# lezhnev74/inverted_index_2

Hardware: NVIDIA B200
Metric: merged postings/s (higher is better)
Workload: dtype u32

## Files before the change

inverted_index_2_b200/csrc/k12_fused.cu:

```cuda
#include "keys.cuh"
#include "union_dev.cuh"

namespace ii2 {

constexpr int F_THREADS = 512;
constexpr int F_MIN_CTAS = 2;
constexpr int F_WARPS = F_THREADS / 32;
constexpr uint32_t F_CAP_I = 1024;
constexpr int F_PER = (F_CAP_I + F_THREADS - 1) / F_THREADS;
constexpr uint32_t F_HT = F_CAP_I > 512 ? 2048 : 1024;
constexpr uint32_t F_A_CH = F_CAP_I * 5 / 4;
constexpr uint32_t F_C_CH = F_CAP_I;
constexpr uint32_t F_B_CH = F_CAP_I * 9 / 8;
constexpr uint32_t F_ARENA_W = (F_A_CH + F_C_CH) * 4;
constexpr uint32_t F_GCAP = F_CAP_I * 4;
constexpr uint32_t F_SMALL_D = 64;
constexpr uint32_t F_EMPTY = 0xFFFFFFFFu;
static_assert(F_CAP_I <= 1024 && F_CAP_I % 64 == 0 && F_THREADS >= 128 && F_THREADS % 32 == 0 &&
              F_HT >= 2 * F_CAP_I, "tile shape");
static_assert(F_B_CH * 16 < 65536, "term positions inside the staged bytes are 16-bit");
static_assert(F_ARENA_W < (1u << 14) && F_GCAP < (1u << 13), "packed output prefixes");

__host__ __device__ inline size_t k12f_smem_bytes(int k) {
  return (size_t)(F_A_CH + F_C_CH + F_B_CH) * 16 + 64
// ... 352 lines not shown
    }
  } else {
    bitonic_sort_any(reps, D, tid, (uint32_t)F_THREADS, less, [] { __syncthreads(); });
    __syncthreads();
    uint32_t run_p = 0, run_e = 0;
    for (uint32_t base = 0; base < D; base += F_THREADS) {
      const uint32_t r = base + tid;
      uint32_t me = 0, li = 0, ei = 0;
      if (r < D) {
        me = reps[r];
        const uint32_t len = cg[me] & 0xFFFFFu;
        if (len > REG_CAP) s_bad = 1;
        li = (len + 3u) & ~3u;
        ei = enc_slot_words(len);
      }
      uint32_t tp, te;
      const uint32_t xp = block_exclusive_scan(li, s_ws32, tp);
      const uint32_t xe = block_exclusive_scan(ei, s_ws32, te);
      if (r < D) {
        order[r] = (uint16_t)me;
        pbase[me] = run_p + xp;
        ebase[me] = run_e + xe;
        if (li >= 128)
          wide_list[atomicAdd(&s_nw, 1u)] = (uint16_t)r;
        else
          narrow_list[atomicAdd(&s_nn, 1u)] = (uint16_t)r;
      }
      run_p += tp;
      run_e += te;
    }
    if (tid == 0) {
      s_tot[0] = run_p;
      s_tot[1] = run_e;
    }
  }
  __syncthreads();
  if (s_bad || s_tot[0] > F_GCAP || (a.want_enc && s_tot[1] > F_ARENA_W)) {
    defer();
    return;
  }

#pragma unroll
  for (int j = 0; j < F_PER; j++) {
    const uint32_t i = tid + j * F_THREADS;
    if (i < W) {
      const uint32_t g = og[j] >> 20;
      const uint32_t* src = reinterpret_cast<const uint32_t*>(smem + ps[j]);
      uint32_t* dst = gather + pbase[g] + (og[j] & 0xFFFFFu);
      const uint32_t n = pl[j];
      uint32_t t = 0;
#pragma unroll 1
      for (; t + 4 <= n; t += 4) {
        const uint32_t x0 = src[t], x1 = src[t + 1], x2 = src[t + 2], x3 = src[t + 3];
        dst[t] = x0;
        dst[t + 1] = x1;
        dst[t + 2] = x2;
        dst[t + 3] = x3;
      }
      if (t < n) {
        const uint32_t x0 = src[t];
        const uint32_t x1 = t + 1 < n ? src[t + 1] : 0u;
        const uint32_t x2 = t + 2 < n ? src[t + 2] : 0u;
        dst[t] = x0;
        if (t + 1 < n) dst[t + 1] = x1;
        if (t + 2 < n) dst[t + 2] = x2;
      }
    }
  }
  __syncthreads();

  uint32_t* const arena = reinterpret_cast<uint32_t*>(smem + OFF_A);
  {
    const unsigned half = lane >> 4, hl = lane & 15u;
    const uint32_t nw = s_nw, nn = s_nn;
    const uint32_t items = nw + ((nn + 1) >> 1);
#pragma unroll 1
    for (uint32_t it = warp; it < items; it += F_WARPS) {
      if (it < nw) {
        const uint32_t r = wide_list[it];
        const uint32_t me = order[r];
        const uint32_t c = cg[me];
        uint32_t* const wslot = gather + pbase[me];
        uint32_t* const weslot = arena + ebase[me];
        const uint32_t outn = union_blocked<32>(wslot, wslot, c & 0xFFFFFu, (c >> 20) > 1, a.rem);
        uint32_t enc = 0;
        if (a.want_enc && outn) enc = encode_shared_warp(wslot, outn, weslot);
        if (lane == 0) rres[r] = outn | (enc << 16);
      } else {
        const uint32_t q = 2 * (it - nw) + half;
        const bool has = q < nn;
        const uint32_t r = has ? narrow_list[q] : 0u;
        const uint32_t me = has ? order[r] : 0u;
        const uint32_t c = has ? cg[me] : 0u;
        uint32_t* const slot = gather + (has ? pbase[me] : 0u);
        uint32_t* const eslot = arena + (has ? ebase[me] : 0u);
        const uint32_t outn = union_blocked<16>(slot, slot, c & 0xFFFFFu, (c >> 20) > 1, a.rem);
        uint32_t enc = 0;
        if (a.want_enc) enc = encode_small_blocked<16>(slot, outn, eslot);
        if (has && hl == 0) rres[r] = outn | (enc << 16);
      }
      __syncwarp();
    }
  }
  __syncthreads();

  const bool keep_empty = a.keep_empty != 0;
  auto packed = [&](uint32_t r) -> uint64_t {
    const uint32_t res = rres[r];
    const uint32_t cnt = res & 0xFFFFu, enc = res >> 16;
    if (!(cnt || keep_empty)) return 0ull;
    return 1ull | ((uint64_t)cnt << 11) | ((uint64_t)enc << 24) | ((uint64_t)tlen[order[r]] << 38);
  };
  if (D <= 64) {
    if (warp == 0) {
      const uint64_t v0 = lane < D ? packed(lane) : 0ull;
      const uint64_t v1 = lane + 32 < D ? packed(lane + 32) : 0ull;
      const uint64_t i0 = warp_inclusive_scan(v0);
      const uint64_t t0 = __shfl_sync(0xffffffffu, i0, 31);
      const uint64_t i1 = warp_inclusive_scan(v1) + t0;
      if (lane < D) pfx[lane] = i0 - v0;
      if (lane + 32 < D) pfx[lane + 32] = i1 - v1;
      if (lane == 31) s_total = i1;
    }
  } else {
    uint64_t run = 0;
    for (uint32_t base = 0; base < D; base += F_THREADS) {
      const uint32_t r = base + tid;
      const uint64_t v = r < D ? packed(r) : 0ull;
      uint64_t tot;
      const uint64_t ex = block_exclusive_scan(v, s_ws64, tot);
      if (r < D) pfx[r] = run + ex;
      run += tot;
    }
    if (tid == 0) s_total = run;
  }
  __syncthreads();
  {
    const uint64_t P0 = a.bk_P[b], E0 = a.bk_E[b], T0 = a.bk_TB[b];
    uint8_t* const o_tb = a.st_tb + T0;
    uint32_t* const o_enc = a.st_enc + E0;
    uint32_t* const o_post = a.st_post + P0;
#pragma unroll 1
    for (uint32_t r = warp; r < D; r += F_WARPS) {
      const uint32_t res = rres[r];
      const uint32_t cnt = res & 0xFFFFu, enc = res >> 16;
      if (!(cnt || keep_empty)) continue;
      const uint32_t me = order[r];
      const uint64_t x = pfx[r];
      const uint32_t t = (uint32_t)x & 0x7FFu, po = (uint32_t)(x >> 11) & 0x1FFFu,
                     eo = (uint32_t)(x >> 24) & 0x3FFFu, to = (uint32_t)(x >> 38);
      const uint32_t n = tlen[me];
      if (lane == 0) {
        a.st_toff[rec_base + t] = to;
        if (a.want_enc) a.st_eoff[rec_base + t] = eo;
        if (a.want_dec) a.st_poff[rec_base + t] = po;
      }
      const uint8_t* tsrc = smem + OFF_B + tsm[me];
      for (uint32_t i = lane; i < n; i += 32) o_tb[to + i] = tsrc[i];
      if (a.want_enc) {
        const uint32_t* esrc = arena + ebase[me];
        for (uint32_t i = lane; i < enc; i += 32) o_enc[eo + i] = esrc[i];
      }
      if (a.want_dec) {
        const uint32_t* dsrc = gather + pbase[me];
        for (uint32_t i = lane; i < cnt; i += 32) o_post[po + i] = dsrc[i];
      }
    }
  }
  if (tid == 0) {
    const uint64_t x = s_total;
    a.bk_D[b] = D;
    a.bk_mode[b] = K12F_DENSE;
    a.bk_raw[0ull * a.nb1 + b] = x & 0x7FFu;
    a.bk_raw[1ull * a.nb1 + b] = x >> 38;
    a.bk_raw[2ull * a.nb1 + b] = (x >> 11) & 0x1FFFu;
    a.bk_raw[3ull * a.nb1 + b] = (x >> 24) & 0x3FFFu;
  }
}

bool k12f_supported(int k) {
  return k >= 1 && k <= (int)F_MAXK && 4 * k <= (int)F_CAP_I && k <= F_THREADS;
// ... 17 lines not shown
```

inverted_index_2_b200/csrc/k12_union.cu:

```cuda
#include <algorithm>
#include <cstdlib>
#include <vector>

#include "intcomp.cuh"
#include "keys.cuh"
#include "union.cuh"
#include "union_dev.cuh"

namespace ii2 {

constexpr int K1B_THREADS = 256;
constexpr int K1B_WARPS = K1B_THREADS / 32;
constexpr uint32_t CAP_I = 1024;
constexpr uint32_t K1B_HT = CAP_I > 512 ? 2048 : 1024;
static_assert(CAP_I % K1B_THREADS == 0 && CAP_I <= 1024 && CAP_I % 4 == 0,
              "tile = a whole number of instances per thread, 10-bit tile indexes");
constexpr uint32_t K1B_STAGE_CAP = CAP_I * 6;
constexpr uint32_t K1B_SMALL_D = 64;
constexpr uint32_t K1B_EMPTY = 0xFFFFFFFFu;
constexpr uint32_t K12_PENDING = 0xFFFFFFFFu;
constexpr uint32_t K1B_HEAVY = 0xFFFFFFFFu;

struct K1bArgs {
  const SegDesc* segs;
// ... 393 lines not shown
      if (tid == 0) {
        s_tot[0] = run_p;
        s_tot[1] = run_e;
      }
    }
    __syncthreads();

    const uint32_t tile_p = s_tot[0];
    const bool staged = tile_p <= K1B_STAGE_CAP;
    uint32_t* const stage = reinterpret_cast<uint32_t*>(key_hi);
    auto copy_source = [](const uint32_t* __restrict__ src, uint32_t* __restrict__ dst, uint32_t n) {
      uint32_t t = 0;
#pragma unroll 1
      for (; t + 4 <= n; t += 4) {
        const uint32_t x0 = __ldg(src + t), x1 = __ldg(src + t + 1), x2 = __ldg(src + t + 2),
                       x3 = __ldg(src + t + 3);
        dst[t] = x0;
        dst[t + 1] = x1;
        dst[t + 2] = x2;
        dst[t + 3] = x3;
      }
      if (t < n) {
        const uint32_t x0 = __ldg(src + t);
        const uint32_t x1 = t + 1 < n ? __ldg(src + t + 1) : 0u;
        const uint32_t x2 = t + 2 < n ? __ldg(src + t + 2) : 0u;
        dst[t] = x0;
        if (t + 1 < n) dst[t + 1] = x1;
        if (t + 2 < n) dst[t + 2] = x2;
      }
    };
#pragma unroll
    for (int j = 0; j < PER; j++) {
      const uint32_t i = tid + j * K1B_THREADS;
      if (i < size) {
        const uint32_t g = og[j] >> 20;
        const uint32_t pb = pbase[g];
        if (pb != K1B_HEAVY) {
          const uint32_t* src = reinterpret_cast<const uint32_t*>(pp[j]);
          const uint32_t at = pb + (og[j] & 0xFFFFFu);
          if (staged)
            copy_source(src, stage + (at - pcount), pl[j]);
          else
            copy_source(src, gath + at, pl[j]);
        } else {
          const uint32_t at = sbase[g] + ((atomicSub(&cg[g], 1u << 20) >> 20) - 1u);
          a.src_ptr[at] = pp[j];
          a.src_len[at] = pl[j];
        }
      }
    }
    if (staged) {
      __syncthreads();
      uint32_t* const out = gath + pcount;
      const uint32_t head = min(tile_p, (uint32_t)((16u - ((uintptr_t)out & 15u)) & 15u) >> 2);
      if (tid < head) out[tid] = stage[tid];
      const uint32_t nvec = (tile_p - head) >> 2;
      for (uint32_t v = tid; v < nvec; v += K1B_THREADS) {
        const uint32_t e = head + 4 * v;
        *reinterpret_cast<uint4*>(out + e) =
            make_uint4(stage[e], stage[e + 1], stage[e + 2], stage[e + 3]);
      }
      const uint32_t tail0 = head + 4 * nvec;
      if (tail0 + tid < tile_p) out[tail0 + tid] = stage[tail0 + tid];
    }
    dcount += D;
    icount += size;
    pcount += s_tot[0];
    ecount += s_tot[1];
    W -= size;
    if (W == 0) break;
    __syncthreads();
    for (int s = tid; s < k; s += K1B_THREADS) cur[s] = mmp[s];
    __syncthreads();
  }
  if (tid == 0) a.bk_D[b] = dcount;
}


constexpr int K2B_THREADS = 128;
constexpr int K2B_WARPS = K2B_THREADS / 32;
constexpr uint32_t K2B_HALF = 128;
constexpr uint32_t K2B_ENC_WORDS = 3 + 2 * 129 + 1 + (5 * 127 + 3) / 4 + 1;
constexpr uint32_t K2B_EBUF = (K2B_ENC_WORDS + 7) & ~7u;
static_assert(K2B_EBUF / 2 >= 1 + (5 * 127 + 3) / 4, "var-byte stream of 127 values fits a half");

struct K2bArgs {
  const uint64_t* bk_pos;
  const uint64_t* bk_P;
  const uint64_t* bk_E;
  const uint32_t* bk_D;
  const GroupIn* gin;
  RemovedSet rem;
  int want_enc, want_dec, keep_empty;
  GroupRec* recs;
  uint32_t* gath;
  uint32_t* tmp_enc;
  uint64_t* bk_raw;
  uint32_t nb1;
  uint32_t* n_large;
  uint32_t* large_rec;
  uint32_t* large_bucket;
  uint32_t bucket0;
  const uint32_t* list;
};

constexpr int K2B_MIN_CTAS = 8;
template <bool LIST>
__global__ void __launch_bounds__(K2B_THREADS, K2B_MIN_CTAS) k2b_union_kernel(const K2bArgs a) {
  pdl_enter();
  __shared__ __align__(16) uint32_t s_buf[K2B_WARPS][REG_CAP];
  __shared__ __align__(16) uint32_t s_enc[K2B_WARPS][K2B_EBUF];
  const unsigned lane = lane_id(), warp = warp_id();
  const unsigned half = lane >> 4, hl = lane & 15u;
  const uint32_t b = LIST ? a.list[blockIdx.x] : a.bucket0 + blockIdx.x;
  const uint32_t D = a.bk_D[b];
  if (D == 0) return;
  const uint64_t rec_base = a.bk_pos[b];
  uint32_t* const gath = a.gath + a.bk_P[b];
  uint32_t* const enc_base = a.tmp_enc + a.bk_E[b];
  uint32_t acc_t = 0, acc_tb = 0, acc_e = 0;
  uint64_t acc_p = 0;
  const GroupIn g_none = {0u, 0u, 0u, 0u, 0u, 0u, 0u, 0u};
  GroupIn g_next = g_none;
  if (2 * warp + half < D) g_next = a.gin[rec_base + 2 * warp + half];
#pragma unroll 1
  for (uint32_t p0 = 2 * warp; p0 < D; p0 += 2 * K2B_WARPS) {
    const uint32_t r = p0 + half;
    const bool has = r < D;
    const GroupIn g = g_next;
    {
      const uint32_t rn = r + 2 * K2B_WARPS;
      g_next = g_none;
      if (rn < D) g_next = a.gin[rec_base + rn];
    }

    const bool heavy = has && g.L > REG_CAP;
    const bool wide = has && !heavy && g.L >= K2B_HALF;
    if (heavy && hl == 0) {
      const uint32_t slot = atomicAdd(a.n_large, 1u);
      a.large_rec[slot] = (uint32_t)(rec_base + r);
      a.large_bucket[slot] = b;
      GroupRec rec;
      rec.inst = g.inst;
      rec.tlen = g.tlen;
      rec.dec = 0;
      rec.eoff = 0;
      rec.enc = 0;
      rec.cnt = K12_PENDING;
      a.recs[rec_base + r] = rec;
    }
    {
      const bool mine = has && !heavy && !wide;
      const uint32_t L = mine ? g.L : 0u;
      uint32_t* const slot = gath + g.pst;
      uint32_t* const buf = s_buf[warp] + half * K2B_HALF;
      uint32_t* const ebuf = s_enc[warp] + half * (K2B_EBUF / 2);
      const uint32_t outn = union_blocked<16>(slot, buf, L, g.c > 1, a.rem);
      if (a.want_dec)
        for (uint32_t e = hl; e < outn; e += 16) slot[e] = buf[e];
      uint32_t enc = 0;
      uint32_t* const enc_dst = enc_base + g.eslot;
      if (a.want_enc) {
        enc = encode_small_blocked<16>(buf, outn, ebuf);
        for (uint32_t e = hl; e < enc; e += 16) enc_dst[e] = ebuf[e];
      }
      if (mine && hl == 0) {
        GroupRec rec;
        rec.inst = g.inst;
        rec.tlen = g.tlen;
        rec.dec = reinterpret_cast<uint64_t>(slot);
        rec.eoff = a.want_enc ? reinterpret_cast<uint64_t>(enc_dst) : 0ull;
        rec.cnt = outn;
        rec.enc = enc;
        a.recs[rec_base + r] = rec;
        if (outn || a.keep_empty) {
          acc_t += 1;
          acc_tb += g.tlen;
          acc_p += outn;
          acc_e += enc;
        }
      }
      __syncwarp();
    }
    unsigned wmask = __ballot_sync(0xffffffffu, wide && hl == 0);
    while (wmask) {
      const int src = __ffs(wmask) - 1;
      wmask &= wmask - 1;
      GroupIn w;
      w.inst = __shfl_sync(0xffffffffu, g.inst, src);
      w.tlen = __shfl_sync(0xffffffffu, g.tlen, src);
      w.c = __shfl_sync(0xffffffffu, g.c, src);
      w.L = __shfl_sync(0xffffffffu, g.L, src);
      w.pst = __shfl_sync(0xffffffffu, g.pst, src);
      w.eslot = __shfl_sync(0xffffffffu, g.eslot, src);
      const uint32_t rw = p0 + (src >> 4);
      uint32_t* const slot = gath + w.pst;
      uint32_t* const buf = s_buf[warp];
      uint32_t* const ebuf = s_enc[warp];
      const uint32_t outn = union_blocked<32>(slot, buf, w.L, w.c > 1, a.rem);
      if (a.want_dec)
        for (uint32_t e = lane; e < outn; e += 32) slot[e] = buf[e];
      uint32_t enc = 0;
      uint32_t* const enc_dst = enc_base + w.eslot;
      if (a.want_enc && outn) {
        enc = encode_shared_warp(buf, outn, ebuf);
        for (uint32_t e = lane; e < enc; e += 32) enc_dst[e] = ebuf[e];
      }
      if (lane == 0) {
        GroupRec rec;
        rec.inst = w.inst;
        rec.tlen = w.tlen;
        rec.dec = reinterpret_cast<uint64_t>(slot);
        rec.eoff = a.want_enc ? reinterpret_cast<uint64_t>(enc_dst) : 0ull;
        rec.cnt = outn;
        rec.enc = enc;
        a.recs[rec_base + rw] = rec;
        if (outn || a.keep_empty) {
          acc_t += 1;
          acc_tb += w.tlen;
          acc_p += outn;
          acc_e += enc;
        }
      }
      __syncwarp();
    }
  }
  if (hl == 0 && acc_t) {
    unsigned long long* bo = reinterpret_cast<unsigned long long*>(a.bk_raw);
    atomicAdd(&bo[0ull * a.nb1 + b], (unsigned long long)acc_t);
    atomicAdd(&bo[1ull * a.nb1 + b], (unsigned long long)acc_tb);
    atomicAdd(&bo[2ull * a.nb1 + b], (unsigned long long)acc_p);
    atomicAdd(&bo[3ull * a.nb1 + b], (unsigned long long)acc_e);
  }
}

constexpr uint32_t MW_CAP = 1024;
constexpr int MW_V = 32;
constexpr int MW_WARPS = 4;
constexpr int MW_MIN_CTAS = 5;
constexpr uint32_t MW_BUF = MW_CAP + MW_CAP / 32 + 8;
constexpr uint32_t MW_EBUF = 3 + 8 * 129 + 1 + 1 + 6;
static_assert(MW_EBUF >= kMaxSegs + 1, "source prefix fits the stream buffer");

struct MwArgs {
  const uint32_t* n_in_list;
  const uint32_t* in_rec;
  const uint32_t* in_bucket;
  const GroupIn* gin;
  const uint64_t* src_ptr;
  const uint32_t* src_len;
  GroupRec* recs;
  RemovedSet rem;
  int want_enc, keep_empty;
  uint64_t* bk_raw;
  uint32_t nb1;
  uint32_t* cursor;
  uint32_t* n_out_list;
  uint32_t* out_rec;
  uint32_t* out_bucket;
  uint32_t* out_post;
  uint32_t* out_enc;
  unsigned long long* out_cursor;
};

__global__ void __launch_bounds__(MW_WARPS * 32, MW_MIN_CTAS) k2_mwarp_kernel(const MwArgs a) {
  pdl_enter();
  __shared__ __align__(16) uint32_t s_buf[MW_WARPS][MW_BUF];
  __shared__ __align__(16) uint32_t s_enc[MW_WARPS][MW_EBUF];
  const unsigned lane = lane_id(), warp = warp_id();
  uint32_t* const buf = s_buf[warp];
  uint32_t* const ebuf = s_enc[warp];
  uint32_t* const moff = ebuf;
  for (;;) {
    uint32_t item = 0;
    if (lane == 0) item = atomicAdd(a.cursor, 1u);
    item = __shfl_sync(0xffffffffu, item, 0);
    if (item >= *a.n_in_list) return;
    const uint32_t rec = a.in_rec[item], bucket = a.in_bucket[item];
    const GroupIn g = a.gin[rec];
    const uint32_t c = g.c, beg = g.src;
    uint32_t run = 0;
    for (uint32_t base = 0; base < c; base += 32) {
      const uint32_t i = base + lane;
      uint32_t li = i < c ? a.src_len[beg + i] : 0u;
      li = li > MW_CAP + 1 ? MW_CAP + 1 : li;
      const uint32_t inc = warp_inclusive_scan(li);
      if (i < c) moff[i] = min(run + inc - li, MW_CAP + 1);
      run = min(run + __shfl_sync(0xffffffffu, inc, 31), MW_CAP + 1);
    }
    if (run > MW_CAP) {
      if (lane == 0) {
        const uint32_t at = atomicAdd(a.n_out_list, 1u);
        a.out_rec[at] = rec;
        a.out_bucket[at] = bucket;
      }
      continue;
// ... 774 lines not shown
  II2_TRY(u.recs.alloc_scratch(N, s));
  II2_TRY(u.bk_D.alloc_scratch(B, s));
  II2_TRY(u.bk_raw.alloc_scratch(4 * (size_t)(B + 1), s));
  II2_TRY(u.bk_out.alloc_scratch(4 * (size_t)(B + 1), s));
  II2_TRY(u.totals.alloc_scratch(8, s));
  const uint64_t enc_cap = n_in + n_in / 4 + 6ull * N + 64;
  if (want_enc) II2_TRY(u.tmp_enc.alloc_scratch(enc_cap, s, 16));
  II2_TRY(u.tmp_post.alloc_scratch(n_in, s, 16));
  const uint32_t large_cap = (uint32_t)std::min<uint64_t>(N, n_in / REG_CAP + 1);
  DevBuf<uint32_t> large_u32;
  II2_TRY(large_u32.alloc_scratch(8 * (size_t)large_cap, s));
  DevBuf<unsigned long long> med_cursor;
  II2_TRY(med_cursor.alloc_scratch(8, s));
  II2_CUDA_TRY(cudaMemsetAsync(med_cursor.p, 0, 64, s));
  II2_TRY(u.med_post.alloc_scratch(n_in, s, 16));
  if (want_enc) II2_TRY(u.med_enc.alloc_scratch(n_in + n_in / 4 + 16ull * large_cap + 64, s, 16));
  II2_CUDA_TRY(cudaMemsetAsync(u.totals.p, 0, 64, s));
  II2_CUDA_TRY(cudaMemsetAsync(u.bk_raw.p, 0, 4 * (size_t)(B + 1) * 8, s));
  II2_TRY(u.bk_mode.alloc_scratch(B, s));
  if (u.fused) {
    II2_TRY(u.st_tb.alloc_scratch(tb_in, s, 64));
    II2_TRY(u.st_off.alloc_scratch(3 * (size_t)N, s));
    II2_TRY(u.def_list.alloc_scratch(B, s));
  } else {
    II2_CUDA_TRY(cudaMemsetAsync(u.bk_mode.p, 0, (size_t)B * 4, s));
  }

  K1bArgs a1;
  a1.segs = plan.segs;
  a1.k = k;
  a1.part = plan.part.p;
  a1.btb = plan.btb.p;
  a1.bpo = plan.bpo.p;
  a1.bk_pos = plan.bk_pos();
  a1.bk_cpl = plan.bk_cpl.p;
  a1.bk_P = plan.bk_P();
  a1.gin = gin.p;
  a1.gath = u.tmp_post.p;
  a1.src_ptr = src_ptr.p;
  a1.src_len = src_len.p;
  a1.bk_D = u.bk_D.p;
  K2bArgs a2;
  a2.bk_pos = plan.bk_pos();
  a2.bk_P = plan.bk_P();
  a2.bk_E = plan.bk_E();
  a2.bk_D = u.bk_D.p;
  a2.gin = gin.p;
  a2.rem = rem;
  a2.want_enc = want_enc ? 1 : 0;
  a2.want_dec = want_dec ? 1 : 0;
  a2.keep_empty = keep_empty ? 1 : 0;
  a2.recs = u.recs.p;
  a2.gath = u.tmp_post.p;
  a2.tmp_enc = u.tmp_enc.p;
  a2.bk_raw = u.bk_raw.p;
  a2.nb1 = B + 1;
  a2.n_large = reinterpret_cast<uint32_t*>(u.totals.p + 6);
  a2.large_rec = large_u32.p;
  a2.large_bucket = large_u32.p + large_cap;
  const size_t smem = k1b_smem_bytes(k);
  static size_t attr = 0;
  if (smem > attr) {
    const size_t want = std::max(k1b_smem_bytes(kMaxSegs), smem);
    II2_CUDA_TRY(cudaFuncSetAttribute(k1b_group_kernel<false>, cudaFuncAttributeMaxDynamicSharedMemorySize,
                                      (int)want));
    II2_CUDA_TRY(cudaFuncSetAttribute(k1b_group_kernel<true>, cudaFuncAttributeMaxDynamicSharedMemorySize,
                                      (int)want));
    attr = want;
  }
  auto general = [&](uint32_t grid, const uint32_t* list) -> int {
    a1.bucket0 = a2.bucket0 = 0;
    a1.list = a2.list = list;
    {
      ProfScope scope("k1b_group", s);
      if (list) {
        II2_LAUNCH_CHAIN(k1b_group_kernel<true>, grid, K1B_THREADS, smem, s, a1);
      } else {
        II2_LAUNCH_CHAIN(k1b_group_kernel<false>, grid, K1B_THREADS, smem, s, a1);
      }
    }
    {
      ProfScope scope("k2b_union", s);
      if (list) {
        II2_LAUNCH_CHAIN(k2b_union_kernel<true>, grid, K2B_THREADS, 0, s, a2);
      } else {
        II2_LAUNCH_CHAIN(k2b_union_kernel<false>, grid, K2B_THREADS, 0, s, a2);
      }
    }
    {
      ProfScope scope("k2_medium", s);
      uint32_t* const mid_rec = large_u32.p + 4 * (size_t)large_cap;
      uint32_t* const mid_bucket = large_u32.p + 5 * (size_t)large_cap;
      uint32_t* const n_mid = reinterpret_cast<uint32_t*>(med_cursor.p + 3);
      MwArgs w2;
      w2.n_in_list = a2.n_large;
      w2.in_rec = a2.large_rec;
      w2.in_bucket = a2.large_bucket;
      w2.gin = gin.p;
      w2.src_ptr = src_ptr.p;
      w2.src_len = src_len.p;
      w2.recs = u.recs.p;
      w2.rem = rem;
      w2.want_enc = want_enc ? 1 : 0;
      w2.keep_empty = keep_empty ? 1 : 0;
      w2.bk_raw = u.bk_raw.p;
      w2.nb1 = B + 1;
      w2.cursor = reinterpret_cast<uint32_t*>(med_cursor.p + 2) + 1;
      w2.n_out_list = n_mid;
      w2.out_rec = mid_rec;
      w2.out_bucket = mid_bucket;
      w2.out_post = u.med_post.p;
      w2.out_enc = u.med_enc.p;
      w2.out_cursor = med_cursor.p;
      II2_LAUNCH_CHAIN(k2_mwarp_kernel, kNumSMs * MW_MIN_CTAS, MW_WARPS * 32, 0, s, w2);
      uint32_t* const mid2_rec = large_u32.p + 6 * (size_t)large_cap;
      uint32_t* const mid2_bucket = large_u32.p + 7 * (size_t)large_cap;
      uint32_t* const n_mid2 = reinterpret_cast<uint32_t*>(med_cursor.p + 3) + 1;
      MedArgs m;
      m.n_large = n_mid;
      m.large_rec = mid_rec;
      m.large_bucket = mid_bucket;
      m.gin = gin.p;
      m.src_ptr = src_ptr.p;
      m.src_len = src_len.p;
      m.recs = u.recs.p;
      m.rem = rem;
      m.want_enc = want_enc ? 1 : 0;
      m.keep_empty = keep_empty ? 1 : 0;
      m.bk_raw = u.bk_raw.p;
      m.nb1 = B + 1;
      m.cursor = reinterpret_cast<uint32_t*>(med_cursor.p + 4);
      m.n_huge = n_mid2;
      m.huge_rec = mid2_rec;
      m.huge_bucket = mid2_bucket;
      m.out_post = u.med_post.p;
      m.out_enc = u.med_enc.p;
      m.out_cursor = med_cursor.p;
      II2_LAUNCH_CHAIN(k2_medium_kernel<4>, kNumSMs * 8, 4 * 32, 0, s, m);
      m.n_large = n_mid2;
      m.large_rec = mid2_rec;
      m.large_bucket = mid2_bucket;
      m.cursor = reinterpret_cast<uint32_t*>(med_cursor.p + 2);
      m.n_huge = a2.n_large + 1;
      m.huge_rec = large_u32.p + 2 * (size_t)large_cap;
      m.huge_bucket = large_u32.p + 3 * (size_t)large_cap;
      II2_LAUNCH_CHAIN(k2_medium_kernel<8>, kNumSMs * 5, 8 * 32, 0, s, m);
    }
    return II2_OK;
  };
  uint64_t* h_tot = pinned_scratch();
  if (!h_tot) return II2_ERR_NOMEM;
  auto totals = [&](bool emit_early = false) -> int {
    ProfScope scope("k12_scan_sync", s);
    II2_TRY(exclusive_scan_multi_sum_to_host(u.bk_raw.p, u.bk_out.p, B + 1, 4, u.totals.p, u.bk_D.p, B,
                                             4, h_tot, 8, s));
    if (emit_early) II2_TRY(k6_emit_early(plan, u, n_in, tb_in, *u.early_out, s));
    II2_CUDA_TRY(cudaStreamSynchronize(s));
    return II2_OK;
  };
  if (u.fused) {
    K12fArgs f;
    f.segs = plan.segs;
    f.k = k;
    f.part = plan.part.p;
    f.btb = plan.btb.p;
    f.bpo = plan.bpo.p;
    f.bk_pos = plan.bk_pos();
    f.bk_cpl = plan.bk_cpl.p;
    f.bk_P = plan.bk_P();
// ... 59 lines not shown
```

inverted_index_2_b200/csrc/union_dev.cuh:

```cuda
#pragma once
#include "intcomp.cuh"
#include "union.cuh"

namespace ii2 {

constexpr uint32_t REG_CAP = 256;

__host__ __device__ __forceinline__ uint32_t enc_slot_words(uint32_t n) { return n + (n >> 2) + 6; }

__device__ __forceinline__ void cex(uint32_t& x, uint32_t& y) {
  const uint32_t lo = min(x, y), hi = max(x, y);
  x = lo;
  y = hi;
}

__device__ __forceinline__ void sort8_local(uint32_t (&v)[8]) {
  cex(v[0], v[1]); cex(v[2], v[3]); cex(v[4], v[5]); cex(v[6], v[7]);
  cex(v[0], v[2]); cex(v[1], v[3]); cex(v[4], v[6]); cex(v[5], v[7]);
  cex(v[1], v[2]); cex(v[5], v[6]); cex(v[0], v[4]); cex(v[3], v[7]);
  cex(v[1], v[5]); cex(v[2], v[6]);
  cex(v[1], v[4]); cex(v[3], v[6]);
  cex(v[2], v[4]); cex(v[3], v[5]);
  cex(v[3], v[4]);
}
// ... 32 lines not shown
  if (nmax > 8) merge_level<16>(v, hl);
  if (nmax > 16) merge_level<32>(v, hl);
  if (nmax > 32) merge_level<64>(v, hl);
  if (nmax > 64) merge_level<128>(v, hl);
  if (W == 32 && nmax > 128) merge_level<256>(v, hl);
}

template <int V>
__device__ __forceinline__ void sort_local_v(uint32_t (&v)[V]) {
#pragma unroll
  for (int k = 2; k <= V; k <<= 1) {
#pragma unroll
    for (int j = k >> 1; j > 0; j >>= 1) {
#pragma unroll
      for (int i = 0; i < V; i++) {
        const int l = i ^ j;
        if (l > i) {
          const uint32_t lo = min(v[i], v[l]), hi = max(v[i], v[l]);
          const bool asc = (i & k) == 0;
          v[i] = asc ? lo : hi;
          v[l] = asc ? hi : lo;
        }
      }
    }
  }
}

template <int V>
__device__ __forceinline__ void clean_local_v(uint32_t (&v)[V]) {
#pragma unroll
  for (int d = V / 2; d > 0; d >>= 1) {
#pragma unroll
    for (int i = 0; i < V; i++)
      if ((i & d) == 0) cex(v[i], v[i + d]);
  }
}

template <int V>
__device__ __forceinline__ void sort_warp_v(uint32_t (&v)[V], unsigned lane, uint32_t n) {
  sort_local_v<V>(v);
#pragma unroll 1
  for (uint32_t K = 2 * V; K <= 32 * V && n > K / 2; K <<= 1) {
    {
      const unsigned dist = K / V - 1;
      const bool lower = (lane & (K / (2 * V))) == 0;
#pragma unroll
      for (int r = 0; r < V / 2; r++) {
        const uint32_t a = v[r], b = v[V - 1 - r];
        const uint32_t oa = __shfl_xor_sync(0xffffffffu, b, dist);
        const uint32_t ob = __shfl_xor_sync(0xffffffffu, a, dist);
        v[r] = ((a < oa) == lower) ? a : oa;
        v[V - 1 - r] = ((b < ob) == lower) ? b : ob;
      }
    }
#pragma unroll 1
    for (uint32_t j = K / 4; j >= V; j >>= 1) {
      const unsigned dist = j / V;
      const bool lower = (lane & dist) == 0;
#pragma unroll
      for (int r = 0; r < V; r++) {
        const uint32_t o = __shfl_xor_sync(0xffffffffu, v[r], dist);
        v[r] = ((v[r] < o) == lower) ? v[r] : o;
      }
    }
    clean_local_v<V>(v);
  }
}

template <int V>
__device__ __forceinline__ void clean_warp_v(uint32_t (&v)[V], unsigned lane) {
#pragma unroll 1
  for (unsigned dist = 16; dist >= 1; dist >>= 1) {
    const bool lower = (lane & dist) == 0;
#pragma unroll
    for (int r = 0; r < V; r++) {
      const uint32_t o = __shfl_xor_sync(0xffffffffu, v[r], dist);
      v[r] = ((v[r] < o) == lower) ? v[r] : o;
    }
  }
  clean_local_v<V>(v);
}

template <int W>
__device__ __forceinline__ uint32_t union_blocked(const uint32_t* slot, uint32_t* buf, uint32_t L,
                                                  bool multi, const RemovedSet& rem) {
  const unsigned lane = lane_id(), hl = lane & (W - 1);
  uint32_t v[8];
#pragma unroll
  for (int r = 0; r < 8; r++) {
    const uint32_t e = hl * 8 + r;
    v[r] = e < L ? slot[e] : 0xFFFFFFFFu;
  }
  const bool any_multi = __any_sync(0xffffffffu, multi && L > 1);
  if (any_multi) {
    const uint32_t nmax = __reduce_max_sync(0xffffffffu, multi ? L : 0u);
    sort_blocked<W>(v, hl, nmax);
    if (!multi) {
#pragma unroll
      for (int r = 0; r < 8; r++) {
        const uint32_t e = hl * 8 + r;
        v[r] = e < L ? slot[e] : 0xFFFFFFFFu;
      }
    }
  }
  uint32_t keep = 0;
  if (rem.bitmap) {
    const uint32_t nbits = (uint32_t)rem.bitmap_bits;
    uint32_t word[8];
#pragma unroll
    for (int r = 0; r < 8; r++) {
      const bool probe = hl * 8 + r < L && v[r] < nbits;
      word[r] = probe ? __ldg(rem.bitmap + (v[r] >> 5)) : 0u;
    }
#pragma unroll
    for (int r = 0; r < 8; r++)
      keep |= (hl * 8 + r < L && !((word[r] >> (v[r] & 31u)) & 1u)) ? 1u << r : 0u;
  } else {
#pragma unroll
    for (int r = 0; r < 8; r++)
      if (hl * 8 + r < L && !is_removed(rem, v[r])) keep |= 1u << r;
  }
  const uint32_t up = __shfl_up_sync(0xffffffffu, v[7], 1, W);
  if (multi) {
    if (hl > 0 && up == v[0]) keep &= ~1u;
#pragma unroll
    for (int r = 1; r < 8; r++)
      if (v[r] == v[r - 1]) keep &= ~(1u << r);
  }
  const uint32_t cnt = __popc(keep);
  uint32_t inc = cnt;
#pragma unroll
  for (int d = 1; d < W; d <<= 1) {
    const uint32_t o = __shfl_up_sync(0xffffffffu, inc, d, W);
    if (hl >= (unsigned)d) inc += o;
  }
  const uint32_t outn = __shfl_sync(0xffffffffu, inc, W - 1, W);
  uint32_t* dst = buf + (inc - cnt);
#pragma unroll
  for (int r = 0; r < 8; r++) {
    const bool k = (keep >> r) & 1u;
    if (k) *dst = v[r];
    dst += k ? 1 : 0;
  }
  __syncwarp();
  return outn;
}

template <int W>
__device__ __forceinline__ uint32_t encode_small_blocked(const uint32_t* v, uint32_t n,
                                                         uint32_t* out) {
  const unsigned hl = lane_id() & (W - 1);
  const uint32_t e0 = hl * 8;
  const uint4 a = *reinterpret_cast<const uint4*>(v + e0);
  const uint4 b = *reinterpret_cast<const uint4*>(v + e0 + 4);
  const uint32_t x[8] = {a.x, a.y, a.z, a.w, b.x, b.y, b.z, b.w};
  uint32_t prev = e0 ? v[e0 - 1] : 0u;
  uint32_t z[8], lens = 0, bytes = 0;
#pragma unroll
  for (int r = 0; r < 8; r++) {
    z[r] = intcomp::zigzag(x[r], prev);
    prev = x[r];
    const uint32_t bl = 32u - __clz(z[r] | 1u);
    const uint32_t len = e0 + r < n ? ((bl + 6u) * 37u) >> 8 : 0u;
    lens |= len << (4 * r);
    bytes += len;
  }
  uint32_t inc = bytes;
#pragma unroll
  for (int d = 1; d < W; d <<= 1) {
    const uint32_t o = __shfl_up_sync(0xffffffffu, inc, d, W);
    if (hl >= (unsigned)d) inc += o;
  }
  const uint32_t total = __shfl_sync(0xffffffffu, inc, W - 1, W);
  uint32_t sb = (uint32_t)__cvta_generic_to_shared(out + 1) + (inc - bytes);
#pragma unroll
  for (int r = 0; r < 8; r++) {
    const uint32_t zz = z[r];
    const uint32_t len = (lens >> (4 * r)) & 15u;
    uint32_t w = (zz & 0x7Fu) | ((zz << 1) & 0x7F00u) | ((zz << 2) & 0x7F0000u) |
                 ((zz << 3) & 0x7F000000u);
    const uint32_t term = 0x80u << ((8 * len - 8) & 31u);
    w |= len <= 4 ? term : 0u;
    const uint32_t b4 = (zz >> 28) | 0x80u;
    asm volatile(
        "{\n\t"
        ".reg .pred p0, p1, p2, p3, p4;\n\t"
        ".reg .b32 t1, t2, t3;\n\t"
        "setp.gt.u32 p0, %1, 0;\n\t"
        "setp.gt.u32 p1, %1, 1;\n\t"
        "setp.gt.u32 p2, %1, 2;\n\t"
        "setp.gt.u32 p3, %1, 3;\n\t"
        "setp.gt.u32 p4, %1, 4;\n\t"
        "shr.u32 t1, %2, 8;\n\t"
        "shr.u32 t2, %2, 16;\n\t"
        "shr.u32 t3, %2, 24;\n\t"
        "@p0 st.shared.u8 [%0], %2;\n\t"
        "@p1 st.shared.u8 [%0+1], t1;\n\t"
        "@p2 st.shared.u8 [%0+2], t2;\n\t"
        "@p3 st.shared.u8 [%0+3], t3;\n\t"
        "@p4 st.shared.u8 [%0+4], %3;\n\t"
        "}"
        :
        : "r"(sb), "r"(len), "r"(w), "r"(b4)
        : "memory");
    sb += len;
  }
  if (n) {
    if (hl == 0) out[0] = n;
    uint8_t* end = reinterpret_cast<uint8_t*>(out + 1) + total;
    if (hl < ((4u - (total & 3u)) & 3u)) end[hl] = 0;
  }
  __syncwarp();
  return n ? 1 + (total + 3) / 4 : 0u;
}

__device__ __forceinline__ uint32_t encode_shared_warp(const uint32_t* v, uint32_t n, uint32_t* out) {
  if (n == 0) return 0;
  const unsigned lane = lane_id();
  const uint32_t nb = n >> 7, tail = n & 127u;
  uint32_t pos = 0;
  if (nb) {
    pos = 3;
#pragma unroll 1
    for (uint32_t blk = 0; blk < nb; blk++) {
      const uint32_t hpos = pos++;
      uint32_t hdr = 0;
#pragma unroll 1
      for (uint32_t g = 0; g < 4; g++) {
        const uint32_t idx = blk * 128 + g * 32 + lane;
        const uint32_t cur = v[idx];
        const uint32_t prev = idx ? v[idx - 1] : cur;
        const uint32_t z = intcomp::zigzag(cur, prev);
        const uint32_t m = __reduce_or_sync(0xffffffffu, z);
        const uint32_t sgn = m & 1u;
        const uint32_t bw = sgn ? intcomp::bitlen(m) : intcomp::bitlen(m >> 1);
        const uint32_t coded = sgn ? z : (cur - prev);
        hdr |= ((sgn << 7) | bw) << (24 - 8 * g);
        if (bw == 32) {
          out[pos + lane] = coded;
        } else if (bw > 0) {
          if (lane < bw) out[pos + lane] = 0;
          __syncwarp();
          const uint32_t bit = lane * bw, sh = bit & 31u;
          atomicOr(&out[pos + (bit >> 5)], coded << sh);
          if (sh + bw > 32u) atomicOr(&out[pos + (bit >> 5) + 1], coded >> (32u - sh));
        }
        pos += bw;
      }
      if (lane == 0) out[hpos] = hdr;
    }
    if (lane == 0) {
      out[0] = nb * 128;
      out[1] = pos;
      out[2] = v[0];
    }
  }
  if (tail) {
    if (lane == 0) out[pos] = tail;
    pos += 1;
    uint8_t* sb = reinterpret_cast<uint8_t*>(out + pos);
    uint32_t bo = 0;
#pragma unroll 1
    for (uint32_t t0 = 0; t0 < tail; t0 += 32) {
      const uint32_t i = t0 + lane;
      uint32_t z = 0, len = 0;
      if (i < tail) {
        const uint32_t idx = nb * 128 + i;
        z = intcomp::zigzag(v[idx], i ? v[idx - 1] : 0u);
        len = intcomp::vbyte_len(z);
      }
      const uint32_t inc = warp_inclusive_scan(len);
      const uint32_t off = bo + inc - len;
      if (len > 0) sb[off] = (uint8_t)((z & 0x7Fu) | (len == 1 ? 0x80u : 0u));
      if (len > 1) sb[off + 1] = (uint8_t)(((z >> 7) & 0x7Fu) | (len == 2 ? 0x80u : 0u));
      if (len > 2) sb[off + 2] = (uint8_t)(((z >> 14) & 0x7Fu) | (len == 3 ? 0x80u : 0u));
      if (len > 3) sb[off + 3] = (uint8_t)(((z >> 21) & 0x7Fu) | (len == 4 ? 0x80u : 0u));
      if (len > 4) sb[off + 4] = (uint8_t)(((z >> 28) & 0x7Fu) | 0x80u);
      bo += __shfl_sync(0xffffffffu, inc, 31);
    }
    if (lane < ((4u - (bo & 3u)) & 3u)) sb[bo + lane] = 0;
    pos += (bo + 3) / 4;
  }
  __syncwarp();
  return pos;
}

constexpr int MED_V = 16;
constexpr uint32_t MED_RUN = 32 * MED_V;
__device__ __forceinline__ uint32_t med_run_slot(uint32_t e) { return e + (e >> 4); }

template <int NW>
__device__ __forceinline__ uint32_t cta_union_term(const uint64_t* __restrict__ g_ptr, uint32_t c,
                                                   uint32_t L, const RemovedSet& rem, uint32_t* s_v,
                                                   uint32_t* s_o, const uint32_t* s_moff,
                                                   uint32_t* s_cnt, uint32_t* s_last) {
  constexpr int MED_THREADS = NW * 32;
// ... 158 lines not shown
```

Measured before the change: 32.70 billion.

## Fuse union dedup with var-byte encoding directly from registers

Splits union_blocked into union_keep (dedup into registers) and compact_blocked, and adds encode_regs. encode_regs zigzag-encodes kept values straight from registers, packs the var-byte codes into 32-bit words and stitches boundary words across lanes with shuffles, replacing byte-wise shared-memory stores. k2b gains an ENC template parameter so the small-group path writes encoded output directly to global instead of staging in shared memory and copying, and drops the gin register double-buffer in favour of a prefetch when encoding. The aim is to cut shared-memory traffic, extra copies and byte stores, at the cost of more complex cross-lane word merging that carries some correctness risk.

```diff
diff --git a/inverted_index_2_b200/csrc/k12_fused.cu b/inverted_index_2_b200/csrc/k12_fused.cu
--- a/inverted_index_2_b200/csrc/k12_fused.cu
+++ b/inverted_index_2_b200/csrc/k12_fused.cu
@@ -458,8 +458,9 @@
         const uint32_t c = cg[me];
         uint32_t* const wslot = gather + pbase[me];
         uint32_t* const weslot = arena + ebase[me];
-        const uint32_t outn = union_blocked<32>(wslot, wslot, c & 0xFFFFFu, (c >> 20) > 1, a.rem);
-        uint32_t enc = 0;
+        uint32_t v[8], enc = 0;
+        const uint32_t keep = union_keep<32>(wslot, c & 0xFFFFFu, (c >> 20) > 1, a.rem, v);
+        const uint32_t outn = compact_blocked<32>(v, keep, wslot);
         if (a.want_enc && outn) enc = encode_shared_warp(wslot, outn, weslot);
         if (lane == 0) rres[r] = outn | (enc << 16);
       } else {
@@ -470,9 +471,10 @@
         const uint32_t c = has ? cg[me] : 0u;
         uint32_t* const slot = gather + (has ? pbase[me] : 0u);
         uint32_t* const eslot = arena + (has ? ebase[me] : 0u);
-        const uint32_t outn = union_blocked<16>(slot, slot, c & 0xFFFFFu, (c >> 20) > 1, a.rem);
-        uint32_t enc = 0;
-        if (a.want_enc) enc = encode_small_blocked<16>(slot, outn, eslot);
+        uint32_t v[8], enc;
+        const uint32_t keep = union_keep<16>(slot, c & 0xFFFFFu, (c >> 20) > 1, a.rem, v);
+        const uint32_t outn = encode_regs<16>(v, keep, a.want_enc ? eslot : nullptr,
+                                              a.want_dec ? slot : nullptr, &enc);
         if (has && hl == 0) rres[r] = outn | (enc << 16);
       }
       __syncwarp();
diff --git a/inverted_index_2_b200/csrc/k12_union.cu b/inverted_index_2_b200/csrc/k12_union.cu
--- a/inverted_index_2_b200/csrc/k12_union.cu
+++ b/inverted_index_2_b200/csrc/k12_union.cu
@@ -499,7 +499,6 @@
 constexpr uint32_t K2B_HALF = 128;
 constexpr uint32_t K2B_ENC_WORDS = 3 + 2 * 129 + 1 + (5 * 127 + 3) / 4 + 1;
 constexpr uint32_t K2B_EBUF = (K2B_ENC_WORDS + 7) & ~7u;
-static_assert(K2B_EBUF / 2 >= 1 + (5 * 127 + 3) / 4, "var-byte stream of 127 values fits a half");
 
 struct K2bArgs {
   const uint64_t* bk_pos;
@@ -522,7 +521,7 @@
 };
 
 constexpr int K2B_MIN_CTAS = 8;
-template <bool LIST>
+template <bool LIST, bool ENC>
 __global__ void __launch_bounds__(K2B_THREADS, K2B_MIN_CTAS) k2b_union_kernel(const K2bArgs a) {
   pdl_enter();
   __shared__ __align__(16) uint32_t s_buf[K2B_WARPS][REG_CAP];
@@ -539,16 +538,21 @@
   uint64_t acc_p = 0;
   const GroupIn g_none = {0u, 0u, 0u, 0u, 0u, 0u, 0u, 0u};
   GroupIn g_next = g_none;
-  if (2 * warp + half < D) g_next = a.gin[rec_base + 2 * warp + half];
+  if (!ENC && 2 * warp + half < D) g_next = a.gin[rec_base + 2 * warp + half];
 #pragma unroll 1
   for (uint32_t p0 = 2 * warp; p0 < D; p0 += 2 * K2B_WARPS) {
     const uint32_t r = p0 + half;
     const bool has = r < D;
-    const GroupIn g = g_next;
+    GroupIn g = g_next;
     {
       const uint32_t rn = r + 2 * K2B_WARPS;
-      g_next = g_none;
-      if (rn < D) g_next = a.gin[rec_base + rn];
+      if (ENC) {
+        g = has ? a.gin[rec_base + r] : g_none;
+        if (rn < D && hl == 0) asm volatile("prefetch.global.L1 [%0];" ::"l"(a.gin + rec_base + rn));
+      } else {
+        g_next = g_none;
+        if (rn < D) g_next = a.gin[rec_base + rn];
+      }
     }
 
     const bool heavy = has && g.L > REG_CAP;
@@ -570,23 +574,20 @@
       const bool mine = has && !heavy && !wide;
       const uint32_t L = mine ? g.L : 0u;
       uint32_t* const slot = gath + g.pst;
+      uint32_t* const enc_dst = enc_base + g.eslot;
       uint32_t* const buf = s_buf[warp] + half * K2B_HALF;
-      uint32_t* const ebuf = s_enc[warp] + half * (K2B_EBUF / 2);
-      const uint32_t outn = union_blocked<16>(slot, buf, L, g.c > 1, a.rem);
-      if (a.want_dec)
+      uint32_t v[8], enc;
+      const uint32_t keep = union_keep<16>(slot, L, g.c > 1, a.rem, v);
+      const uint32_t outn = encode_regs<16>(v, keep, ENC ? enc_dst : nullptr,
+                                            a.want_dec ? (ENC ? slot : buf) : nullptr, &enc);
+      if (!ENC && a.want_dec)
         for (uint32_t e = hl; e < outn; e += 16) slot[e] = buf[e];
-      uint32_t enc = 0;
-      uint32_t* const enc_dst = enc_base + g.eslot;
-      if (a.want_enc) {
-        enc = encode_small_blocked<16>(buf, outn, ebuf);
-        for (uint32_t e = hl; e < enc; e += 16) enc_dst[e] = ebuf[e];
-      }
       if (mine && hl == 0) {
         GroupRec rec;
         rec.inst = g.inst;
         rec.tlen = g.tlen;
         rec.dec = reinterpret_cast<uint64_t>(slot);
-        rec.eoff = a.want_enc ? reinterpret_cast<uint64_t>(enc_dst) : 0ull;
+        rec.eoff = ENC ? reinterpret_cast<uint64_t>(enc_dst) : 0ull;
         rec.cnt = outn;
         rec.enc = enc;
         a.recs[rec_base + r] = rec;
@@ -612,14 +613,15 @@
       w.eslot = __shfl_sync(0xffffffffu, g.eslot, src);
       const uint32_t rw = p0 + (src >> 4);
       uint32_t* const slot = gath + w.pst;
+      uint32_t* const enc_dst = enc_base + w.eslot;
       uint32_t* const buf = s_buf[warp];
       uint32_t* const ebuf = s_enc[warp];
-      const uint32_t outn = union_blocked<32>(slot, buf, w.L, w.c > 1, a.rem);
+      uint32_t v[8], enc = 0;
+      const uint32_t keep = union_keep<32>(slot, w.L, w.c > 1, a.rem, v);
+      const uint32_t outn = compact_blocked<32>(v, keep, buf);
       if (a.want_dec)
         for (uint32_t e = lane; e < outn; e += 32) slot[e] = buf[e];
-      uint32_t enc = 0;
-      uint32_t* const enc_dst = enc_base + w.eslot;
-      if (a.want_enc && outn) {
+      if (ENC && outn) {
         enc = encode_shared_warp(buf, outn, ebuf);
         for (uint32_t e = lane; e < enc; e += 32) enc_dst[e] = ebuf[e];
       }
@@ -628,7 +630,7 @@
         rec.inst = w.inst;
         rec.tlen = w.tlen;
         rec.dec = reinterpret_cast<uint64_t>(slot);
-        rec.eoff = a.want_enc ? reinterpret_cast<uint64_t>(enc_dst) : 0ull;
+        rec.eoff = ENC ? reinterpret_cast<uint64_t>(enc_dst) : 0ull;
         rec.cnt = outn;
         rec.enc = enc;
         a.recs[rec_base + rw] = rec;
@@ -1569,9 +1571,11 @@
     {
       ProfScope scope("k2b_union", s);
       if (list) {
-        II2_LAUNCH_CHAIN(k2b_union_kernel<true>, grid, K2B_THREADS, 0, s, a2);
+        if (want_enc) II2_LAUNCH_CHAIN((k2b_union_kernel<true, true>), grid, K2B_THREADS, 0, s, a2);
+        else II2_LAUNCH_CHAIN((k2b_union_kernel<true, false>), grid, K2B_THREADS, 0, s, a2);
       } else {
-        II2_LAUNCH_CHAIN(k2b_union_kernel<false>, grid, K2B_THREADS, 0, s, a2);
+        if (want_enc) II2_LAUNCH_CHAIN((k2b_union_kernel<false, true>), grid, K2B_THREADS, 0, s, a2);
+        else II2_LAUNCH_CHAIN((k2b_union_kernel<false, false>), grid, K2B_THREADS, 0, s, a2);
       }
     }
     {
diff --git a/inverted_index_2_b200/csrc/union_dev.cuh b/inverted_index_2_b200/csrc/union_dev.cuh
--- a/inverted_index_2_b200/csrc/union_dev.cuh
+++ b/inverted_index_2_b200/csrc/union_dev.cuh
@@ -138,10 +138,9 @@
 }
 
 template <int W>
-__device__ __forceinline__ uint32_t union_blocked(const uint32_t* slot, uint32_t* buf, uint32_t L,
-                                                  bool multi, const RemovedSet& rem) {
+__device__ __forceinline__ uint32_t union_keep(const uint32_t* slot, uint32_t L, bool multi,
+                                               const RemovedSet& rem, uint32_t (&v)[8]) {
   const unsigned lane = lane_id(), hl = lane & (W - 1);
-  uint32_t v[8];
 #pragma unroll
   for (int r = 0; r < 8; r++) {
     const uint32_t e = hl * 8 + r;
@@ -183,6 +182,13 @@
     for (int r = 1; r < 8; r++)
       if (v[r] == v[r - 1]) keep &= ~(1u << r);
   }
+  return keep;
+}
+
+template <int W>
+__device__ __forceinline__ uint32_t compact_blocked(const uint32_t (&v)[8], uint32_t keep,
+                                                    uint32_t* dst) {
+  const unsigned hl = lane_id() & (W - 1);
   const uint32_t cnt = __popc(keep);
   uint32_t inc = cnt;
 #pragma unroll
@@ -191,83 +197,120 @@
     if (hl >= (unsigned)d) inc += o;
   }
   const uint32_t outn = __shfl_sync(0xffffffffu, inc, W - 1, W);
-  uint32_t* dst = buf + (inc - cnt);
-#pragma unroll
-  for (int r = 0; r < 8; r++) {
-    const bool k = (keep >> r) & 1u;
-    if (k) *dst = v[r];
-    dst += k ? 1 : 0;
+  if (dst) {
+    dst += inc - cnt;
+#pragma unroll
+    for (int r = 0; r < 8; r++) {
+      const bool k = (keep >> r) & 1u;
+      if (k) *dst = v[r];
+      dst += k ? 1 : 0;
+    }
   }
   __syncwarp();
   return outn;
 }
 
+__device__ __forceinline__ uint32_t shl_clamped(uint32_t x, uint32_t sh) {
+  uint32_t r;
+  asm("shl.b32 %0, %1, %2;" : "=r"(r) : "r"(x), "r"(sh));
+  return r;
+}
+
+template <bool FIVE>
+__device__ __forceinline__ void pack_codes(const uint32_t (&z)[8], uint32_t lens, uint32_t* out,
+                                           uint32_t& bit, uint32_t& a0, uint32_t& head,
+                                           bool& first) {
+#pragma unroll
+  for (int r = 0; r < 8; r++) {
+    const uint32_t zz = z[r], len = (lens >> (4 * r)) & 15u;
+    const uint32_t lo = (zz & 0x7Fu) | ((zz << 1) & 0x7F00u) | ((zz << 2) & 0x7F0000u) |
+                        ((zz << 3) & 0x7F000000u) | shl_clamped(0x80u, 8 * len - 8);
+    const uint32_t at = bit >> 5, nb = bit & 31u;
+    a0 |= lo << nb;
+    const uint32_t full = (nb + 8 * len) >> 5;
+    if (FIVE) {
+      const uint32_t t = zz >> 28;
+      const uint32_t hi = t | ((t + 127u) & 0x80u);
+      const uint32_t a1 = __funnelshift_l(lo, hi, nb);
+      const uint32_t a2 = __funnelshift_l(hi, 0u, nb);
+      if (full && !first) out[at] = a0;
+      if (full > 1) out[at + 1] = a1;
+      head = full && first ? a0 : head;
+      first = first && !full;
+      a0 = full > 1 ? a2 : full ? a1 : a0;
+    } else {
+      const uint32_t a1 = __funnelshift_l(lo, 0u, nb);
+      if (full && !first) out[at] = a0;
+      head = full && first ? a0 : head;
+      first = first && !full;
+      a0 = full ? a1 : a0;
+    }
+    bit += 8 * len;
+  }
+}
+
 template <int W>
-__device__ __forceinline__ uint32_t encode_small_blocked(const uint32_t* v, uint32_t n,
-                                                         uint32_t* out) {
-  const unsigned hl = lane_id() & (W - 1);
-  const uint32_t e0 = hl * 8;
-  const uint4 a = *reinterpret_cast<const uint4*>(v + e0);
-  const uint4 b = *reinterpret_cast<const uint4*>(v + e0 + 4);
-  const uint32_t x[8] = {a.x, a.y, a.z, a.w, b.x, b.y, b.z, b.w};
-  uint32_t prev = e0 ? v[e0 - 1] : 0u;
+__device__ __forceinline__ uint32_t encode_regs(const uint32_t (&v)[8], uint32_t keep,
+                                                uint32_t* out, uint32_t* dec, uint32_t* words) {
+  const unsigned lane = lane_id(), hl = lane & (W - 1);
+  if (dec || !out) {
+    const uint32_t n = compact_blocked<W>(v, keep, dec);
+    *words = 0;
+    if (!out) return n;
+  }
   uint32_t z[8], lens = 0, bytes = 0;
-#pragma unroll
-  for (int r = 0; r < 8; r++) {
-    z[r] = intcomp::zigzag(x[r], prev);
-    prev = x[r];
-    const uint32_t bl = 32u - __clz(z[r] | 1u);
-    const uint32_t len = e0 + r < n ? ((bl + 6u) * 37u) >> 8 : 0u;
-    lens |= len << (4 * r);
-    bytes += len;
-  }
-  uint32_t inc = bytes;
+  {
+    uint32_t last = 0;
+#pragma unroll
+    for (int r = 0; r < 8; r++) last = (keep >> r) & 1u ? v[r] : last;
+    const unsigned grp = W == 32 ? 0xffffffffu : 0xffffu << (lane & 16u);
+    const unsigned below = __ballot_sync(0xffffffffu, keep != 0) & grp & ((1u << lane) - 1u);
+    const uint32_t from = __shfl_sync(0xffffffffu, last, (31 - __clz(below)) & 31);
+    uint32_t prev = below ? from : 0u;
+#pragma unroll
+    for (int r = 0; r < 8; r++) {
+      const uint32_t km = 0u - ((keep >> r) & 1u);
+      const uint32_t zz = intcomp::zigzag(v[r], prev);
+      prev = km ? v[r] : prev;
+      z[r] = zz & km;
+      const uint32_t len = (((38u - __clz(zz | 1u)) * 37u) >> 8) & km;
+      lens |= len << (4 * r);
+      bytes += len;
+    }
+  }
+  const uint32_t mine = __popc(keep) | bytes << 16;
+  uint32_t inc = mine;
 #pragma unroll
   for (int d = 1; d < W; d <<= 1) {
     const uint32_t o = __shfl_up_sync(0xffffffffu, inc, d, W);
     if (hl >= (unsigned)d) inc += o;
   }
-  const uint32_t total = __shfl_sync(0xffffffffu, inc, W - 1, W);
-  uint32_t sb = (uint32_t)__cvta_generic_to_shared(out + 1) + (inc - bytes);
-#pragma unroll
-  for (int r = 0; r < 8; r++) {
-    const uint32_t zz = z[r];
-    const uint32_t len = (lens >> (4 * r)) & 15u;
-    uint32_t w = (zz & 0x7Fu) | ((zz << 1) & 0x7F00u) | ((zz << 2) & 0x7F0000u) |
-                 ((zz << 3) & 0x7F000000u);
-    const uint32_t term = 0x80u << ((8 * len - 8) & 31u);
-    w |= len <= 4 ? term : 0u;
-    const uint32_t b4 = (zz >> 28) | 0x80u;
-    asm volatile(
-        "{\n\t"
-        ".reg .pred p0, p1, p2, p3, p4;\n\t"
-        ".reg .b32 t1, t2, t3;\n\t"
-        "setp.gt.u32 p0, %1, 0;\n\t"
-        "setp.gt.u32 p1, %1, 1;\n\t"
-        "setp.gt.u32 p2, %1, 2;\n\t"
-        "setp.gt.u32 p3, %1, 3;\n\t"
-        "setp.gt.u32 p4, %1, 4;\n\t"
-        "shr.u32 t1, %2, 8;\n\t"
-        "shr.u32 t2, %2, 16;\n\t"
-        "shr.u32 t3, %2, 24;\n\t"
-        "@p0 st.shared.u8 [%0], %2;\n\t"
-        "@p1 st.shared.u8 [%0+1], t1;\n\t"
-        "@p2 st.shared.u8 [%0+2], t2;\n\t"
-        "@p3 st.shared.u8 [%0+3], t3;\n\t"
-        "@p4 st.shared.u8 [%0+4], %3;\n\t"
-        "}"
-        :
-        : "r"(sb), "r"(len), "r"(w), "r"(b4)
-        : "memory");
-    sb += len;
-  }
-  if (n) {
-    if (hl == 0) out[0] = n;
-    uint8_t* end = reinterpret_cast<uint8_t*>(out + 1) + total;
-    if (hl < ((4u - (total & 3u)) & 3u)) end[hl] = 0;
-  }
-  __syncwarp();
-  return n ? 1 + (total + 3) / 4 : 0u;
+  const uint32_t tot = __shfl_sync(0xffffffffu, inc, W - 1, W);
+  if ((tot & 0xFFFFu) && hl == 0) out[0] = tot & 0xFFFFu;
+
+  const uint32_t off = (inc - mine) >> 16;
+  const uint32_t key = (off >> 2) & 255u;
+  uint32_t bit = 32 + 8 * off;
+  uint32_t a0 = (off & 3u) ? key : 0u, head = key;
+  bool first = (off & 3u) != 0;
+  if (__any_sync(0xffffffffu, (lens >> 2) & lens & 0x11111111u))
+    pack_codes<true>(z, lens, out, bit, a0, head, first);
+  else
+    pack_codes<false>(z, lens, out, bit, a0, head, first);
+  if (__any_sync(0xffffffffu, (tot & 0xFFFFu) != 0)) {
+    uint32_t acc = first ? a0 : head;
+#pragma unroll
+    for (int d = 1; d < W; d <<= 1) {
+      const uint32_t o = __shfl_down_sync(0xffffffffu, acc, d, W);
+      if (((o ^ acc) & 255u) == 0) acc |= o;
+    }
+    const uint32_t above = __shfl_down_sync(0xffffffffu, acc, 1, W);
+    if (!first && (bit & 31u))
+      out[bit >> 5] = a0 | ((lane_id() & (W - 1)) + 1 < W ? above & ~255u : 0u);
+  }
+  const uint32_t n = tot & 0xFFFFu;
+  *words = n ? 1 + ((tot >> 16) + 3) / 4 : 0u;
+  return n;
 }
 
 __device__ __forceinline__ uint32_t encode_shared_warp(const uint32_t* v, uint32_t n, uint32_t* out) {
```

Result: faster. 33.34 billion (median of 6 runs) (+1.9%).
